# openai/blocksparse

Measured on AMD Instinct MI355X. Metric: bsmm_effective_tflops_4096x4096_bs32_d20, higher is better.
Workload: dtype bf16

## Files before the change

blocksparse_amd/csrc/bsmm_xflow.h:

```cpp
#pragma once
#include "bsmm_common.h"
#include "bsmm_plan.h"
#include "bsmm_updat_v2.h"
#include "bsmm_updat_tr.h"
#include "bsmm_xprop.h"

namespace bsmm {

#ifndef X4_NO_XDMA
#define X4_NO_XDMA 0
#endif
#ifndef X4_NO_WDMA
#define X4_NO_WDMA 0
#endif
#ifndef X4_NO_MATH
#define X4_NO_MATH 0
#endif
#ifndef X4_READS_FIRST
#define X4_READS_FIRST 1
#endif
#ifndef X4_PUBLISH_FIRST
#define X4_PUBLISH_FIRST 1
#endif
#ifndef X4_FETCH_EARLY
#define X4_FETCH_EARLY 0
#endif
#ifndef X4_STAGGER
#define X4_STAGGER 0
#endif
#ifndef X4_PRIO
#define X4_PRIO 0
#endif
#ifdef X4_TIMELINE
__device__ unsigned long long g_x4_tl[256 * 40];
#define X4_TL(step, k) do { if (blockIdx.x == 0 && (step) < 256) { const unsigned long long t_ = __builtin_readcyclecounter(); if (lane == 0) g_x4_tl[(step) * 40 + (k)] = t_; } } while (0)
#else
#define X4_TL(step, k) do { } while (0)
#endif
#ifdef X4_STAMPS
__device__ unsigned long long g_x4_trace[64 * 16 * 8];
#define X4_T0() const unsigned long long t0_ = __builtin_readcyclecounter()
#define X4_T1(k) tacc[k] += __builtin_readcyclecounter() - t0_
#else
#define X4_T0() do { } while (0)
#define X4_T1(k) do { } while (0)
#endif
constexpr int X4_R = 128;
constexpr int X4_SLAB = X4_R * 128;
constexpr int X4_S = 2;
constexpr int X4_WBASE = X4_D * X4_SLAB;
constexpr int X4_WWAVE = X4_S * 2048;
constexpr int X4_FLAGS = X4_WBASE + X4_G * X4_WWAVE;
constexpr int X4_LDS = X4_FLAGS + 64 + 64;
constexpr int X4_DI = 16 / X4_PARTS;
static_assert(X4_LDS <= 163840, "flow kernel: ring must fit the LDS");
static_assert(X4_WWAVE >= 64 * 64, "the epilogue stages 64 rows x 64 B per pass in a wave's weight slots");
static_assert((X4_WWAVE & (X4_WWAVE - 1)) == 0 && X4_WBASE % X4_WWAVE == 0, "weight slot toggling by XOR needs aligned slots");

__device__ __forceinline__ void x4_lane_write(uint64_t em, uint32_t v_addr, uint32_t v_value) {
    asm volatile("s_mov_b64 exec, %0\n\tds_write_b32 %1, %2\n\ts_mov_b64 exec, -1" ::"s"(em), "v"(v_addr), "v"(v_value) : "memory");
}
__device__ __forceinline__ void x4_lane_add(uint64_t em, uint32_t v_addr, uint32_t v_value) {
    asm volatile("s_mov_b64 exec, %0\n\tds_add_u32 %1, %2\n\ts_mov_b64 exec, -1" ::"s"(em), "v"(v_addr), "v"(v_value) : "memory");
}
__device__ __forceinline__ void x4_lane_poll_ge(uint64_t em, uint32_t v_addr, uint32_t v_target) {
    uint32_t t;
    asm volatile("s_mov_b64 exec, %1\n"
                 "1:\n\tds_read_b32 %0, %2\n\ts_waitcnt lgkmcnt(0)\n\tv_cmp_ge_u32 vcc, %0, %3\n\ts_cbranch_vccnz 2f\n\ts_sleep 1\n\ts_branch 1b\n"
                 "2:\n\ts_mov_b64 exec, -1"
                 : "=&v"(t) : "s"(em), "v"(v_addr), "v"(v_target) : "memory", "vcc");
}
__device__ __forceinline__ void x4_poll_all_ge(uint32_t v_addr, uint32_t s_need) {
    uint32_t t;
    asm volatile("1:\n\tds_read_b32 %0, %1\n\ts_waitcnt lgkmcnt(0)\n\tv_cmp_gt_u32 vcc, %2, %0\n\ts_cbranch_vccz 2f\n\ts_sleep 1\n\ts_branch 1b\n2:"
                 : "=&v"(t) : "v"(v_addr), "s"(s_need) : "memory", "vcc");
}

#ifndef X4_XPOL
#define X4_XPOL ""
#endif
__device__ __forceinline__ void x4_glds_x(const void* sbase, uint32_t voff, uint32_t lds_byte_addr) {
    unsigned keep;
    asm volatile("s_mov_b32 %0, m0\n\ts_mov_b32 m0, %3\n\ts_nop 0\n\tglobal_load_lds_dwordx4 %1, %2" X4_XPOL "\n\ts_mov_b32 m0, %0"
                 : "=&s"(keep) : "v"(voff), "s"(sbase), "s"(lds_byte_addr) : "memory");
}
__device__ __forceinline__ void x4_glds_x4(const void* sbase, uint32_t v0, uint32_t v1, uint32_t v2, uint32_t v3, uint32_t lds_byte_addr) {
    unsigned keep;
    asm volatile("s_mov_b32 %0, m0\n\ts_mov_b32 m0, %6\n\ts_nop 0\n\tglobal_load_lds_dwordx4 %1, %5" X4_XPOL "\n\t"
                 "s_add_u32 m0, m0, 0x400\n\ts_nop 0\n\tglobal_load_lds_dwordx4 %2, %5" X4_XPOL "\n\t"
                 "s_add_u32 m0, m0, 0x400\n\ts_nop 0\n\tglobal_load_lds_dwordx4 %3, %5" X4_XPOL "\n\t"
                 "s_add_u32 m0, m0, 0x400\n\ts_nop 0\n\tglobal_load_lds_dwordx4 %4, %5" X4_XPOL "\n\ts_mov_b32 m0, %0"
                 : "=&s"(keep) : "v"(v0), "v"(v1), "v"(v2), "v"(v3), "s"(sbase), "s"(lds_byte_addr) : "memory", "scc");
}

template <int DI>
__device__ __forceinline__ void x4_wait_ctl(uint32_t ctl) {
    asm volatile("s_bitcmp1_b32 %0, 3\n\ts_cbranch_scc0 1f\n\ts_waitcnt vmcnt(2)\n\ts_branch 3f\n"
                 "1:\n\ts_bitcmp1_b32 %0, 4\n\ts_cbranch_scc0 2f\n\ts_waitcnt vmcnt(0)\n\ts_branch 3f\n"
                 "2:\n\ts_waitcnt vmcnt(%1)\n3:" ::"s"(ctl), "n"(DI) : "memory", "scc");
}

#ifdef X4_ENDSTAMPS
__device__ unsigned long long g_x4_ends[512 * 16 * 8];
#endif
template <class DT, bool TRANSW, int RT = 4>
__global__ void __launch_bounds__(64 * X4_G, 4)
xflow32_kernel(const typename DT::T* __restrict__ X, const typename DT::T* __restrict__ Wsel, typename DT::T* __restrict__ Y,
               const int32_t* __restrict__ plan, XMap map, int N, int Cin, int Kout) {
    typedef typename DT::T T;
    static_assert(DT::is16, "flow kernel: 16-bit storage types");
    static_assert(RT == 4 || RT == 2, "flow kernel: units of 128 or 64 rows");
    constexpr int R = 32 * RT, SLAB = R * 128, D = X4_D * 4 / RT, DI = X4_DI * RT / 4;
    static_assert(D * SLAB == X4_WBASE && DI % 4 == 0 && D <= 16, "flow kernel: ring geometry");
    extern __shared__ __attribute__((aligned(16))) unsigned char smem[];
    const int lane = threadIdx.x & 63;
    const int wave = __builtin_amdgcn_readfirstlane(threadIdx.x >> 6);
    const int r = lane & 31, h = lane >> 5;
    const uint32_t base_addr = lds_addr_of(smem);
    const uint32_t prog_addr = base_addr + X4_FLAGS, full_addr = base_addr + X4_FLAGS + 64;
    if (threadIdx.x < 32) reinterpret_cast<uint32_t*>(smem + X4_FLAGS)[threadIdx.x] = 0u;
    __syncthreads();
#if X4_STAGGER
    for (int i = ((blockIdx.x >> 3) & 31) * X4_STAGGER; i > 0; --i) __builtin_amdgcn_s_sleep(1);
#endif

    const int npairs_full = Cin / 64;
    const unsigned char* xt = reinterpret_cast<const unsigned char*>(X);
    const unsigned char* wsel = static_cast<const unsigned char*>(uniform_ptr(Wsel));
    const uint32_t wvoff = TRANSW ? (uint32_t)lane * 16u : (uint32_t)((lane >> 2) * 64 + (((lane & 3) ^ ((lane >> 4) & 3)) << 4));
    const uint32_t wslot0 = X4_WBASE + wave * X4_WWAVE;
    const int xsw = (r >> 1) & 7;
    uint32_t xrd[2], wrd[2];
#pragma unroll
    for (int kk = 0; kk < 2; ++kk) {
        xrd[kk] = r * 128 + (((2 * kk + h) ^ xsw) << 4);
        if constexpr (TRANSW) {
            const int g16 = lane >> 4, t16 = lane & 15;
            wrd[kk] = wslot0 + (16 * kk + 8 * h + (t16 >> 2)) * 64 + (16 * (g16 & 1) + 4 * (t16 & 3)) * 2;
        } else {
            wrd[kk] = wslot0 + r * 64 + (((2 * kk + h) ^ ((r >> 2) & 3)) << 4);
        }
    }
    const uint32_t my_prog_s = prog_addr + 4 * wave;
    const uint32_t stride16 = (uint32_t)Cin * 16u;
    const uint32_t pc_e = (uint32_t)((lane & 7) ^ (lane >> 4));
    const uint32_t vo_e = (uint32_t)(lane >> 3) * (uint32_t)Cin * 2u + pc_e * 16u;

#ifdef X4_STAMPS
    unsigned long long tacc[8] = {0, 0, 0, 0, 0, 0, 0, 0};
    const unsigned long long tstart = __builtin_readcyclecounter();
#endif
#ifdef X4_ENDSTAMPS
    int x4e_u = 0;
    if (lane == 0 && blockIdx.x < 512) g_x4_ends[(blockIdx.x * 16 + wave) * 8] = __builtin_amdgcn_s_memrealtime();
#endif
    uint32_t gs = 0;
    const int nunits = map.grid();
    for (int unit = blockIdx.x; unit < nunits; unit += gridDim.x) {
        int tile, grp;
        if (!xmap_decode(map, unit, tile, grp)) continue;
        const int32_t* gh = plan + plan[5] + X4_GROUP * grp;
        const int step_off = __builtin_amdgcn_readfirstlane(gh[0]), nsteps = __builtin_amdgcn_readfirstlane(gh[1]);
        const int list_off = __builtin_amdgcn_readfirstlane(gh[4]), lcap = __builtin_amdgcn_readfirstlane(gh[5]);
        const int32_t* pairs = plan + plan[6] + step_off;
        const int32_t* lists = plan + plan[7] + list_off;
        const int nev = __builtin_amdgcn_readfirstlane(lists[wave]);
        const int my_ob = __builtin_amdgcn_readfirstlane(lists[X4_G + wave]);
        const int32_t* mine = lists + 2 * X4_G + (size_t)2 * lcap * wave;
        const int n_tile = tile * R;
        const unsigned char* xtile = static_cast<const unsigned char*>(uniform_ptr(xt + (size_t)n_tile * Cin * 2));
        const bool fast_tile = n_tile + R <= N;

        f32x16 acc[RT];
#pragma unroll
        for (int t = 0; t < RT; ++t)
#pragma unroll
            for (int i = 0; i < 16; ++i) acc[t][i] = 0.f;

        uint32_t s_w = 0, s_wf = 0;
        for (int eb = 0; eb < nev; eb += 64) {
            const int ei = min(eb + lane, nev - 1);
            const uint32_t w0 = (uint32_t)mine[2 * ei], w1 = (uint32_t)mine[2 * ei + 1];
            const uint32_t ty = w0 & 3, hp = (w0 >> 2) & 3, step = (w0 >> 4) & 0xfff, nxt = (w0 >> 16) & 0xfff;
            const uint32_t gstep = gs + step, sm = gstep % (uint32_t)D, guse = gstep / (uint32_t)D + 1u;
            uint32_t p128 = 0;
            if (ty == 2) p128 = (uint32_t)pairs[step];
            asm volatile("s_waitcnt vmcnt(0)" ::: "memory");
            const uint32_t wn = w1 >> 27;
            const uint32_t f27 = w1 & X4_NOFETCH;
            uint32_t v_ctl = ty | (wn >= (uint32_t)X4_DI ? 0u : (wn >= 2u ? 8u : 16u)) | (f27 != X4_NOFETCH ? 64u : 0u) |
                             ((ty == 2 && (!fast_tile || (int)p128 >= npairs_full)) ? 128u : 0u);
            uint32_t v_x = ty == 1 ? ((sm * (uint32_t)SLAB) | (hp << 6)) : (sm * (uint32_t)SLAB + hp * (uint32_t)(DI * 1024));
            uint32_t v_fa = ty == 2 ? p128 * 128u : full_addr + 4 * sm;
            uint32_t v_g = ty == 2 ? gstep + 1u : guse * (uint32_t)X4_PARTS;
            uint32_t v_pv = gs + nxt;
            uint32_t v_fw = f27 << 11;
            asm volatile("" : "+v"(v_ctl), "+v"(v_x), "+v"(v_fa), "+v"(v_g), "+v"(v_pv), "+v"(v_fw));
#ifdef X4_TIMELINE
            const uint32_t v_dbg = gstep | (hp << 16);
#endif
            const int nchunk = min(64, nev - eb);
            for (int idx = 0; idx < nchunk; ++idx) {
                const uint64_t em = 1ull << idx;
                const uint32_t ctl = (uint32_t)__builtin_amdgcn_readlane(v_ctl, idx);
                const uint32_t ty_s = ctl & 3;
#ifdef X4_STAMPS
                tacc[7] += 1;
#endif
                bool fetched = false;
                if (ty_s & 1) { X4_T0(); x4_wait_ctl<DI>(ctl); X4_T1(0); }
                if (ty_s == 1) {
                    { X4_T0(); x4_lane_poll_ge(em, v_fa, v_g); X4_T1(1); }
#ifdef X4_TIMELINE
                    const uint32_t dbg_s = (uint32_t)__builtin_amdgcn_readlane(v_dbg, idx) & 0xffff;
                    X4_TL(dbg_s, 6 + 2 * wave);
#endif
                    X4_T0();
                    if (X4_PRIO) __builtin_amdgcn_s_setprio(3);
                    if (!X4_NO_MATH) {
                        const uint32_t sx = (uint32_t)__builtin_amdgcn_readlane(v_x, idx);
                        uint4 wq[2];
#pragma unroll
                        for (int kk = 0; kk < 2; ++kk) {
                            if constexpr (TRANSW) {
                                const uint2 lo = ds_tr16(smem + (wrd[kk] ^ s_w)), hi = ds_tr16(smem + (wrd[kk] ^ s_w) + 4 * 64);
                                wq[kk] = make_uint4(lo.x, lo.y, hi.x, hi.y);
                            } else {
                                wq[kk] = *reinterpret_cast<const uint4*>(smem + (wrd[kk] ^ s_w));
                            }
                        }
#if X4_READS_FIRST
                        uint4 xf[RT];
#pragma unroll
                        for (int t = 0; t < RT; ++t) xf[t] = *reinterpret_cast<const uint4*>(smem + (xrd[0] ^ sx) + t * 4096);
                        __builtin_amdgcn_sched_barrier(0);
#pragma unroll
                        for (int t = 0; t < RT; ++t) {
                            acc[t] = DT::mfma32(wq[0], xf[t], acc[t]);
                            xf[t] = *reinterpret_cast<const uint4*>(smem + (xrd[1] ^ sx) + t * 4096);
                            __builtin_amdgcn_sched_barrier(0);
#if X4_FETCH_EARLY
                            if (t == 0 && (ctl & 64u)) {
                                if (!X4_NO_WDMA) {
                                    const uint32_t fo = (uint32_t)__builtin_amdgcn_readlane(v_fw, idx);
                                    glds16_saddr_x2(wsel, wvoff + fo, wvoff + fo + 1024u, base_addr + (wslot0 ^ s_wf));
                                }
                                s_wf ^= 2048u;
                                fetched = true;
                            }
#endif
                        }
#pragma unroll
                        for (int t = 0; t < RT; ++t) acc[t] = DT::mfma32(wq[1], xf[t], acc[t]);
#else
                        uint4 xf[RT][2];
#pragma unroll
                        for (int kk = 0; kk < 2; ++kk)
#pragma unroll
                            for (int t = 0; t < RT; ++t) xf[t][kk] = *reinterpret_cast<const uint4*>(smem + (xrd[kk] ^ sx) + t * 4096);
#pragma unroll
                        for (int kk = 0; kk < 2; ++kk)
#pragma unroll
                            for (int t = 0; t < RT; ++t) acc[t] = DT::mfma32(wq[kk], xf[t][kk], acc[t]);
#endif
                    }
                    s_w ^= 2048u;
#ifdef X4_STAMPS
                    asm volatile("s_nop 0" ::"v"(acc[0][0]), "v"(acc[RT - 1][0]));
#endif
                    X4_T1(2);
#ifdef X4_TIMELINE
                    asm volatile("s_nop 0" ::"v"(acc[0][0]), "v"(acc[RT - 1][0]));
                    X4_TL(dbg_s, 7 + 2 * wave);
#endif
                } else if (ty_s == 2) {
                    const uint32_t g1 = (uint32_t)__builtin_amdgcn_readlane(v_g, idx);
                    { X4_T0(); if (g1 > (uint32_t)D) x4_poll_all_ge(prog_addr + 4 * (lane & 15), g1 - (uint32_t)D); X4_T1(3); }
                    X4_T0();
#ifdef X4_TIMELINE
                    const uint32_t dbg_r = (uint32_t)__builtin_amdgcn_readlane(v_dbg, idx);
                    X4_TL(dbg_r & 0xffff, dbg_r >> 16);
#endif
                    if (!X4_NO_XDMA) {
                        const uint32_t dst = base_addr + (uint32_t)__builtin_amdgcn_readlane(v_x, idx);
                        const uint32_t poff = (uint32_t)__builtin_amdgcn_readlane(v_fa, idx);
                        const uint32_t part_i = (uint32_t)__builtin_amdgcn_readlane(v_x, idx) % (uint32_t)SLAB / 1024u;
                        if (!(ctl & 128u)) {
                            const uint32_t k0 = part_i * stride16 + poff;
                            const uint32_t vo_o = (pc_e & 4u) ? vo_e - 64u : vo_e + 64u;
#pragma unroll
                            for (int k = 0; k < DI; k += 4)
                                x4_glds_x4(xtile, vo_e + (k0 + (k + 0) * stride16), vo_o + (k0 + (k + 1) * stride16), vo_e + (k0 + (k + 2) * stride16),
                                                vo_o + (k0 + (k + 3) * stride16), dst + k * 1024);
                        } else {
                            const bool tail = (int)(poff >> 7) >= npairs_full;
#pragma unroll
                            for (int k = 0; k < DI; ++k) {
                                const int row = 8 * ((int)part_i + k) + (lane >> 3);
                                const int xr = min(n_tile + row, N - 1) - n_tile;
                                const int piece = (lane & 7) ^ ((row >> 1) & 7);
                                uint32_t voff = (uint32_t)xr * (uint32_t)Cin * 2u + piece * 16 + poff;
                                if (tail && (piece & 4)) voff -= 64;
                                x4_glds_x(xtile, voff, dst + k * 1024);
                            }
                        }
                    }
                    X4_T1(4);
#ifdef X4_TIMELINE
                    X4_TL(dbg_r & 0xffff, 2 + (dbg_r >> 16));
#endif
                } else if (ty_s == 3) {
                    x4_lane_add(em, v_fa, 1u);
#ifdef X4_TIMELINE
                    { const uint32_t dbg_a = (uint32_t)__builtin_amdgcn_readlane(v_dbg, idx); X4_TL(dbg_a & 0xffff, 4 + (dbg_a >> 16)); }
#endif
                }
                if (ty_s < 2) {
                    X4_T0();
                    if (X4_PUBLISH_FIRST) x4_lane_write(em, my_prog_s, v_pv);
                    if ((ctl & 64u) && !fetched) {
                        if (!X4_NO_WDMA) {
                            const uint32_t fo = (uint32_t)__builtin_amdgcn_readlane(v_fw, idx);
                            glds16_saddr_x2(wsel, wvoff + fo, wvoff + fo + 1024u, base_addr + (wslot0 ^ s_wf));
                        }
                        s_wf ^= 2048u;
                    }
                    if (!X4_PUBLISH_FIRST) x4_lane_write(em, my_prog_s, v_pv);
                    if (X4_PRIO) __builtin_amdgcn_s_setprio(0);
                    X4_T1(5);
                }
            }
        }
        gs += (uint32_t)nsteps;

        if (my_ob >= 0) {
            unsigned char* stage = smem + wslot0;
            unsigned char* ybase = reinterpret_cast<unsigned char*>(Y + (size_t)my_ob * 32);
#pragma unroll
            for (int pass = 0; pass < RT / 2; ++pass) {
#pragma unroll
                for (int tt = 0; tt < 2; ++tt) {
                    const int t = 2 * pass + tt;
                    const int n = tt * 32 + r;
#pragma unroll
                    for (int q = 0; q < 4; ++q) {
                        const uint32_t lo = (uint32_t)DT::from_f32(acc[t][4 * q + 0]) | ((uint32_t)DT::from_f32(acc[t][4 * q + 1]) << 16);
                        const uint32_t hi = (uint32_t)DT::from_f32(acc[t][4 * q + 2]) | ((uint32_t)DT::from_f32(acc[t][4 * q + 3]) << 16);
                        *reinterpret_cast<uint2*>(stage + n * 64 + ((q ^ ((n >> 2) & 3)) << 4) + 8 * h) = make_uint2(lo, hi);
                    }
                }
                asm volatile("" ::: "memory");
#pragma unroll
                for (int i = 0; i < 4; ++i) {
                    const int n = 16 * i + (lane >> 2), pc = lane & 3;
                    const uint4 v = *reinterpret_cast<const uint4*>(stage + n * 64 + ((pc ^ ((n >> 2) & 3)) << 4));
                    const int gn = n_tile + 64 * pass + n;
                    if (gn < N) *reinterpret_cast<uint4*>(ybase + (size_t)gn * Kout * 2 + pc * 16) = v;
                }
                asm volatile("" ::: "memory");
            }
        }
#ifdef X4_ENDSTAMPS
        if (lane == 0 && blockIdx.x < 512 && x4e_u < 6) g_x4_ends[(blockIdx.x * 16 + wave) * 8 + 1 + x4e_u] = __builtin_amdgcn_s_memrealtime();
        ++x4e_u;
#endif
    }
#ifdef X4_ENDSTAMPS
    if (lane == 0 && blockIdx.x < 512) g_x4_ends[(blockIdx.x * 16 + wave) * 8 + 7] = (unsigned long long)x4e_u;
#endif
#ifdef X4_STAMPS
    tacc[6] = __builtin_readcyclecounter() - tstart;
    if (blockIdx.x < 64 && lane == 0)
        for (int k = 0; k < 8; ++k) g_x4_trace[(blockIdx.x * 16 + wave) * 8 + k] = tacc[k];
#endif
}

}
```

Measured before the change: 700.4.

## Batch readiness polling via ready mask, hoist weight LDS reads, use immediate offsets

Replaces the per-event single-lane LDS poll with a wave-wide ready mask. One poll loop now checks every pending math lane's counter at once and stops only when the current lane is ready, so later events that are already satisfied skip polling. It also moves the weight LDS reads ahead of the readiness wait to hide their latency. It uses immediate offsets on global_load_lds instead of m0 increments for the X and W DMA, which cuts scalar instructions and nops. The risks are extra scalar register pressure and weight reads issued before the sync, which relies on the weight slot already being valid at that point.

Result: no change. 696.4 (-0.6%).

```diff
diff --git a/blocksparse_amd/csrc/bsmm_xflow.h b/blocksparse_amd/csrc/bsmm_xflow.h
--- a/blocksparse_amd/csrc/bsmm_xflow.h
+++ b/blocksparse_amd/csrc/bsmm_xflow.h
@@ -24,6 +24,15 @@
 #endif
 #ifndef X4_FETCH_EARLY
 #define X4_FETCH_EARLY 0
+#endif
+#ifndef X4_READY_MASK
+#define X4_READY_MASK 1
+#endif
+#ifndef X4_WREADS_EARLY
+#define X4_WREADS_EARLY 1
+#endif
+#ifndef X4_IMM_STEP
+#define X4_IMM_STEP 1
 #endif
 #ifndef X4_STAGGER
 #define X4_STAGGER 0
@@ -70,6 +79,15 @@
                  "2:\n\ts_mov_b64 exec, -1"
                  : "=&v"(t) : "s"(em), "v"(v_addr), "v"(v_target) : "memory", "vcc");
 }
+__device__ __forceinline__ uint64_t x4_ready_refresh(uint64_t ready, uint64_t bmask, uint32_t idx, uint32_t v_addr, uint32_t v_target) {
+    uint32_t t;
+    asm volatile("s_mov_b64 exec, %2\n"
+                 "1:\n\tds_read_b32 %1, %4\n\ts_waitcnt lgkmcnt(0)\n\tv_cmp_ge_u32 vcc, %1, %5\n\ts_or_b64 %0, %0, vcc\n\ts_bitcmp1_b64 %0, %3\n\t"
+                 "s_cbranch_scc1 2f\n\ts_sleep 1\n\ts_branch 1b\n"
+                 "2:\n\ts_mov_b64 exec, -1"
+                 : "+s"(ready), "=&v"(t) : "s"(bmask), "s"(idx), "v"(v_addr), "v"(v_target) : "memory", "vcc", "scc");
+    return ready;
+}
 __device__ __forceinline__ void x4_poll_all_ge(uint32_t v_addr, uint32_t s_need) {
     uint32_t t;
     asm volatile("1:\n\tds_read_b32 %0, %1\n\ts_waitcnt lgkmcnt(0)\n\tv_cmp_gt_u32 vcc, %2, %0\n\ts_cbranch_vccz 2f\n\ts_sleep 1\n\ts_branch 1b\n2:"
@@ -91,6 +109,24 @@
                  "s_add_u32 m0, m0, 0x400\n\ts_nop 0\n\tglobal_load_lds_dwordx4 %3, %5" X4_XPOL "\n\t"
                  "s_add_u32 m0, m0, 0x400\n\ts_nop 0\n\tglobal_load_lds_dwordx4 %4, %5" X4_XPOL "\n\ts_mov_b32 m0, %0"
                  : "=&s"(keep) : "v"(v0), "v"(v1), "v"(v2), "v"(v3), "s"(sbase), "s"(lds_byte_addr) : "memory", "scc");
+}
+__device__ __forceinline__ void x4_glds_x4i(const void* sbase, uint32_t v0, uint32_t v1m, uint32_t v2m, uint32_t v3m, uint32_t lds_byte_addr) {
+    unsigned keep;
+    asm volatile("s_mov_b32 %0, m0\n\ts_mov_b32 m0, %6\n\ts_nop 0\n\tglobal_load_lds_dwordx4 %1, %5" X4_XPOL "\n\t"
+                 "global_load_lds_dwordx4 %2, %5 offset:1024" X4_XPOL "\n\t"
+                 "global_load_lds_dwordx4 %3, %5 offset:2048" X4_XPOL "\n\t"
+                 "global_load_lds_dwordx4 %4, %5 offset:3072" X4_XPOL "\n\ts_mov_b32 m0, %0"
+                 : "=&s"(keep) : "v"(v0), "v"(v1m), "v"(v2m), "v"(v3m), "s"(sbase), "s"(lds_byte_addr) : "memory");
+}
+__device__ __forceinline__ void x4_glds_w2(const void* sbase, uint32_t voff, uint32_t lds_byte_addr) {
+#if X4_IMM_STEP
+    unsigned keep;
+    asm volatile("s_mov_b32 %0, m0\n\ts_mov_b32 m0, %3\n\ts_nop 0\n\tglobal_load_lds_dwordx4 %1, %2\n\t"
+                 "global_load_lds_dwordx4 %1, %2 offset:1024\n\ts_mov_b32 m0, %0"
+                 : "=&s"(keep) : "v"(voff), "s"(sbase), "s"(lds_byte_addr) : "memory");
+#else
+    glds16_saddr_x2(sbase, voff, voff + 1024u, lds_byte_addr);
+#endif
 }
 
 template <int DI>
@@ -200,6 +236,10 @@
             const uint32_t v_dbg = gstep | (hp << 16);
 #endif
             const int nchunk = min(64, nev - eb);
+#if X4_READY_MASK
+            const uint64_t bmask = __builtin_amdgcn_ballot_w64(ty == 1 && lane < nchunk);
+            uint64_t ready = 0;
+#endif
             for (int idx = 0; idx < nchunk; ++idx) {
                 const uint64_t em = 1ull << idx;
                 const uint32_t ctl = (uint32_t)__builtin_amdgcn_readlane(v_ctl, idx);
@@ -210,16 +250,8 @@
                 bool fetched = false;
                 if (ty_s & 1) { X4_T0(); x4_wait_ctl<DI>(ctl); X4_T1(0); }
                 if (ty_s == 1) {
-                    { X4_T0(); x4_lane_poll_ge(em, v_fa, v_g); X4_T1(1); }
-#ifdef X4_TIMELINE
-                    const uint32_t dbg_s = (uint32_t)__builtin_amdgcn_readlane(v_dbg, idx) & 0xffff;
-                    X4_TL(dbg_s, 6 + 2 * wave);
-#endif
-                    X4_T0();
-                    if (X4_PRIO) __builtin_amdgcn_s_setprio(3);
-                    if (!X4_NO_MATH) {
-                        const uint32_t sx = (uint32_t)__builtin_amdgcn_readlane(v_x, idx);
-                        uint4 wq[2];
+                    uint4 wq[2];
+                    auto read_wq = [&]() {
 #pragma unroll
                         for (int kk = 0; kk < 2; ++kk) {
                             if constexpr (TRANSW) {
@@ -229,6 +261,37 @@
                                 wq[kk] = *reinterpret_cast<const uint4*>(smem + (wrd[kk] ^ s_w));
                             }
                         }
+                    };
+                    if (X4_WREADS_EARLY && !X4_NO_MATH) read_wq();
+                    {
+                    X4_T0();
+#if X4_READY_MASK
+                    if (!(ready & em)) {
+                        ready = x4_ready_refresh(ready, bmask, (uint32_t)idx, v_fa, v_g);
+#ifdef X4_STAMPS
+                        tacc[7] += 1ull << 40;
+#endif
+                    }
+#else
+                    x4_lane_poll_ge(em, v_fa, v_g);
+#ifdef X4_STAMPS
+                    tacc[7] += 1ull << 40;
+#endif
+#endif
+                    X4_T1(1);
+                    }
+#ifdef X4_STAMPS
+                    tacc[7] += 1ull << 20;
+#endif
+#ifdef X4_TIMELINE
+                    const uint32_t dbg_s = (uint32_t)__builtin_amdgcn_readlane(v_dbg, idx) & 0xffff;
+                    X4_TL(dbg_s, 6 + 2 * wave);
+#endif
+                    X4_T0();
+                    if (X4_PRIO) __builtin_amdgcn_s_setprio(3);
+                    if (!X4_NO_MATH) {
+                        const uint32_t sx = (uint32_t)__builtin_amdgcn_readlane(v_x, idx);
+                        if (!X4_WREADS_EARLY) read_wq();
 #if X4_READS_FIRST
                         uint4 xf[RT];
 #pragma unroll
@@ -243,7 +306,7 @@
                             if (t == 0 && (ctl & 64u)) {
                                 if (!X4_NO_WDMA) {
                                     const uint32_t fo = (uint32_t)__builtin_amdgcn_readlane(v_fw, idx);
-                                    glds16_saddr_x2(wsel, wvoff + fo, wvoff + fo + 1024u, base_addr + (wslot0 ^ s_wf));
+                                    x4_glds_w2(wsel, wvoff + fo, base_addr + (wslot0 ^ s_wf));
                                 }
                                 s_wf ^= 2048u;
                                 fetched = true;
@@ -289,9 +352,15 @@
                             const uint32_t k0 = part_i * stride16 + poff;
                             const uint32_t vo_o = (pc_e & 4u) ? vo_e - 64u : vo_e + 64u;
 #pragma unroll
-                            for (int k = 0; k < DI; k += 4)
+                            for (int k = 0; k < DI; k += 4) {
+#if X4_IMM_STEP
+                                const uint32_t kb = k0 + k * stride16, s16m = stride16 - 1024u;
+                                x4_glds_x4i(xtile, vo_e + kb, vo_o + (kb + s16m), vo_e + (kb + 2 * s16m), vo_o + (kb + 3 * s16m), dst + k * 1024);
+#else
                                 x4_glds_x4(xtile, vo_e + (k0 + (k + 0) * stride16), vo_o + (k0 + (k + 1) * stride16), vo_e + (k0 + (k + 2) * stride16),
                                                 vo_o + (k0 + (k + 3) * stride16), dst + k * 1024);
+#endif
+                            }
                         } else {
                             const bool tail = (int)(poff >> 7) >= npairs_full;
 #pragma unroll
@@ -321,7 +390,7 @@
                     if ((ctl & 64u) && !fetched) {
                         if (!X4_NO_WDMA) {
                             const uint32_t fo = (uint32_t)__builtin_amdgcn_readlane(v_fw, idx);
-                            glds16_saddr_x2(wsel, wvoff + fo, wvoff + fo + 1024u, base_addr + (wslot0 ^ s_wf));
+                            x4_glds_w2(wsel, wvoff + fo, base_addr + (wslot0 ^ s_wf));
                         }
                         s_wf ^= 2048u;
                     }
```
